# vincenthz/eccoxide

Hardware: AMD Instinct MI355X
Metric: variable-base scalarmuls/sec (batch) per GPU + achieved HBM GB/s vs roofline (higher is better)
Workload: dtype u32

## Files before the change

### eccoxide_amd/csrc/eccx_api.cpp

```cpp
#include "../../include/eccx.h"

#include <hip/hip_runtime.h>

#include <algorithm>
#include <cstring>
#include <mutex>
#include <string>
#include <thread>
#include <vector>

#include "launch.hpp"

namespace {

using eccx::CurveOps;

constexpr int NCURVES = 6;
constexpr uint32_t K_BASE_IS_GENERATOR = 1u << 0;
constexpr uint32_t K_OUT_TABLE = 1u << 1;
constexpr uint32_t K_VALIDATE = 1u << 2;
constexpr uint32_t K_OUT_ROWS = 1u << 3;
constexpr uint32_t K_NEGATE_B = 1u << 5;
constexpr uint32_t K_CT_SCAN = 1u << 6;
constexpr uint32_t K_ONLY_MARKED = 1u << 7;
// ... 153 lines not shown
size_t ed_slab_bytes(size_t n) { return 2 * align16(n * 32) + align16(n) + align16(n * 64) + n * 64; }
int ensure_ed(eccx_ctx* ctx, size_t n, EdSlab* out) {
  const int rc = grow_slab(ctx, &ctx->ed, &ctx->ed_cap, ed_slab_bytes(n));
  if (rc || !out) return rc;
  out->u1 = ctx->ed;
  out->u2 = out->u1 + align16(n * 32);
  out->lflags = out->u2 + align16(n * 32);
  out->keys = out->lflags + align16(n);
  out->pts = out->keys + align16(n * 64);
  return ECCX_OK;
}

int norm_grid(const eccx_ctx* ctx, size_t n) {
  size_t tile = (size_t)eccx::LAUNCH_WG * 8;
  size_t tiles = (n + tile - 1) / tile;
  return (int)std::max<size_t>(1, std::min(tiles, (size_t)ctx->cus * 4));
}

int flat_grid(const eccx_ctx* ctx, size_t n) {
  size_t need = (n + eccx::LAUNCH_WG - 1) / eccx::LAUNCH_WG;
  return (int)std::max<size_t>(1, std::min(need, (size_t)ctx->cus * 8));
}

int launch_var(eccx_ctx* ctx, const CurveOps* ops, size_t n, const uint8_t* d_scalars, const uint8_t* d_points,
               uint8_t* d_out, uint8_t* d_flags, uint8_t* d_proj, uint32_t kopts, bool mirror, hipStream_t s,
               bool glv = false, bool ct = false, bool ct_prime = false) {
  if (n == 0) return ECCX_OK;
  if (ct && ops->var_ct && !d_proj && d_points && !(kopts & (K_OUT_TABLE | K_BASE_IS_GENERATOR))) {
    const bool ed = ops->info.edwards != 0;
    const bool prime = ct_prime && ops->var_ct_prime;
    const int grid = prime ? ops->var_ct_prime_grid(ctx->cus, n) : ops->var_ct_grid(ctx->cus, n);
    const int grid2 = std::min(ops->var_grid ? ops->var_grid(ctx->cus, n) : grid_for(ctx, n), ctx->cus);
    int rc = ensure_scratch(ctx, ed ? ops->info.row5_words : ops->coz_row_words, grid);
    if (rc) return rc;
    if (!ed) {
      rc = ensure_scratch(ctx, ops->info.row_words, grid2);
      if (rc) return rc;
    }
    rc = ensure_rows(ctx, ops, n);
    if (rc) return rc;
    HIP_TRY(ctx, (prime ? ops->var_ct_prime : ops->var_ct)(grid, s, n, d_scalars, d_points, ctx->jac, d_flags, ctx->scratch,
                                                           kopts & ~K_CT_SCAN));
    HIP_TRY(ctx, ops->to_affine_var(norm_grid(ctx, n), s, n, ctx->jac, d_out, d_flags));
    if (!ed)
      HIP_TRY(ctx, ops->var(grid2, s, n, d_scalars, d_points, d_out, d_flags, nullptr, ctx->scratch,
                            (kopts & K_VALIDATE) | K_CT_SCAN | K_ONLY_MARKED));
    return ECCX_OK;
  }
  const bool fast = !mirror && ops->var_fast && !d_proj && !(kopts & K_OUT_TABLE);
  if (fast && ops->var_coz && d_points && !(kopts & K_BASE_IS_GENERATOR)) {
    const int g = (glv || ops->var_glv_default) ? 1 : 0;
    const int grid = ops->var_coz_grid(ctx->cus, n, g);
    const int grid2 = ops->var_fast_grid ? ops->var_fast_grid(ctx->cus, n) : grid_for(ctx, n);
    int rc = ensure_scratch(ctx, ops->coz_row_words, grid);
    if (rc) return rc;
    rc = ensure_scratch(ctx, ops->info.row5_words, grid2);
    if (rc) return rc;
    rc = ensure_rows(ctx, ops, n);
    if (rc) return rc;
    HIP_TRY(ctx, ops->var_coz(grid, s, n, d_scalars, d_points, ctx->jac, d_flags, ctx->scratch, kopts, g));
    HIP_TRY(ctx, ops->var_fast(grid2, s, n, d_scalars, d_points, ctx->jac, d_flags, ctx->scratch, kopts | K_ONLY_MARKED));
    HIP_TRY(ctx, ops->to_affine_var(norm_grid(ctx, n), s, n, ctx->jac, d_out, d_flags));
    return ECCX_OK;
  }
  int grid = fast ? (ops->var_fast_grid ? ops->var_fast_grid(ctx->cus, n) : grid_for(ctx, n))
                  : (ops->var_grid ? ops->var_grid(ctx->cus, n) : grid_for(ctx, n));
  if (fast) {
    int rc = ensure_scratch(ctx, ops->info.row5_words, grid);
    if (rc) return rc;
    rc = ensure_rows(ctx, ops, n);
    if (rc) return rc;
    HIP_TRY(ctx, ops->var_fast(grid, s, n, d_scalars, d_points, ctx->jac, d_flags, ctx->scratch, kopts));
    HIP_TRY(ctx, ops->to_affine_var(norm_grid(ctx, n), s, n, ctx->jac, d_out, d_flags));
    return ECCX_OK;
  }
  if (ops->info.row_words) {
    int rc = ensure_scratch(ctx, ops->info.row_words, grid);
    if (rc) return rc;
  }
  if (!d_proj && !(kopts & K_OUT_TABLE) && ops->to_affine_hom) {
    int rc = ensure_rows(ctx, ops, n);
    if (rc) return rc;
    HIP_TRY(ctx, ops->var(grid, s, n, d_scalars, d_points, reinterpret_cast<uint8_t*>(ctx->jac), d_flags, nullptr,
                          ctx->scratch, kopts | K_OUT_ROWS));
    HIP_TRY(ctx, ops->to_affine_hom(norm_grid(ctx, n), s, n, ctx->jac, d_out, d_flags));
    return ECCX_OK;
  }
  HIP_TRY(ctx, ops->var(grid, s, n, d_scalars, d_points, d_out, d_flags, d_proj, ctx->scratch, kopts));
  return ECCX_OK;
}

std::vector<uint8_t> comb_scalars(const CurveOps* ops) {
  int sb = ops->info.sb, nw = 2 * sb;
  std::vector<uint8_t> k((size_t)nw * 16 * sb, 0);
  for (int w = 0; w < nw; ++w)
    for (int d = 0; d < 16; ++d) {
      uint8_t* row = k.data() + ((size_t)w * 16 + d) * sb;
      row[sb - 1 - w / 2] = (uint8_t)((w & 1) ? (d << 4) : d);
    }
  return k;
}

struct DevMem {
  std::vector<void*> ptrs;
  ~DevMem() {
    for (void* p : ptrs)
      if (p) (void)hipFree(p);
// ... 229 lines not shown
    prev_done = done; prev_lo = lo; prev_cnt = cnt;
  }
  TRY2_(copy_out(prev_lo, prev_cnt, prev_done));
  TRY2_(hipStreamSynchronize(s_out));
  if (s_out != ctx->stream) TRY2_(hipStreamSynchronize(ctx->stream));
#undef TRY2_
  return ECCX_OK;
}
template <class Launch>
int host_pipeline(eccx_ctx* ctx, size_t n, const HostIn* ins, int nins, const HostOut* outs, int nouts, bool chunked,
                  Launch launch) {
  return host_pipeline_x(ctx, n, ins, nins, outs, nouts, chunked, launch, [](size_t, size_t, hipStream_t) { return hipSuccess; });
}

int run_host(eccx_ctx* ctx, int curve, bool base, size_t n, const uint8_t* scalars, const uint8_t* points,
             uint8_t* out, uint8_t* flags, uint8_t* proj, uint32_t opts) {
  const CurveOps* ops = ops_of(curve);
  if (!ctx) return ECCX_ERR_ARG;
  if (!ops) return curve_err(ctx);
  if (n == 0) return ECCX_OK;
  if (!scalars || !out || !flags || (!base && !points)) return arg_err(ctx, "null buffer");
  HIP_TRY(ctx, hipSetDevice(ctx->device));
  size_t sb = ops->info.sb, pb = 2 * (size_t)ops->info.fb;
  uint8_t *d_k = nullptr, *d_p = nullptr, *d_o = nullptr, *d_f = nullptr, *d_j = nullptr;
  int rc = ensure_io(ctx, IO_K, n * sb, &d_k);
  if (!rc) rc = ensure_io(ctx, IO_O, n * pb, &d_o);
  if (!rc) rc = ensure_io(ctx, IO_F, n, &d_f);
  if (!rc && !base) rc = ensure_io(ctx, IO_P, n * pb, &d_p);
  if (!rc && proj) rc = ensure_io(ctx, IO_J, n * proj_bytes(ops), &d_j);
  if (rc) return rc;
  const bool chunked = !proj && (!base || ((opts & ECCX_CT_SCAN) && !(opts & (ECCX_MIRROR_REFERENCE | ECCX_TABLE_IN_L2))));
  const HostIn ins[2] = {{d_k, scalars, sb}, {d_p, base ? nullptr : points, pb}};
  const HostOut outs[3] = {{out, d_o, pb}, {flags, d_f, 1}, {proj, d_j, proj_bytes(ops)}};
  return host_pipeline(ctx, n, ins, 2, outs, 3, chunked, [&](size_t lo, size_t cnt) {
    if (base) return eccx_scalarmul_base_dev(ctx, curve, cnt, d_k + lo * sb, d_o + lo * pb, d_f + lo, d_j, opts, ctx->stream);
    return eccx_scalarmul_var_dev(ctx, curve, cnt, d_k + lo * sb, d_p + lo * pb, d_o + lo * pb, d_f + lo, d_j, opts, ctx->stream);
  });
}

int verify_shape(eccx_ctx* ctx, int curve, const CurveOps* ops, size_t n, const uint8_t* d_u1, const uint8_t* d_u2,
                 const uint8_t* d_q, uint8_t* d_out, uint8_t* d_flags, uint32_t opts, hipStream_t s) {
  HIP_TRY(ctx, hipSetDevice(ctx->device));
  int rc = ensure_comb(ctx, curve, ops, s);
  if (rc) return rc;
  if (!ctx->comb_u[curve]) return ECCX_ERR_HIP;
  const int grid = ops->var_fast_grid ? ops->var_fast_grid(ctx->cus, n) : grid_for(ctx, n);
  rc = ensure_scratch(ctx, ops->info.row5_words, grid);
  if (rc) return rc;
  rc = ensure_rows(ctx, ops, n);
  if (rc) return rc;
  const uint32_t kopts = kopts_of(opts) | ((opts & ECCX_SUBTRACT) ? K_NEGATE_B : 0u);
  if (ops->var_coz_fused) {
    const int gridc = ops->var_coz_fused_grid(ctx->cus, n);
    rc = ensure_scratch(ctx, ops->coz_row_words, gridc);
    if (rc) return rc;
    HIP_TRY(ctx, ops->var_coz_fused(gridc, s, n, d_u2, d_q, ctx->jac, d_flags, ctx->scratch, kopts, d_u1, ctx->comb_u[curve]));
  }
  HIP_TRY(ctx, ops->var_fused(grid, s, n, d_u2, d_q, ctx->jac, d_flags, ctx->scratch,
                              kopts | (ops->var_coz_fused ? K_ONLY_MARKED : 0u), d_u1, ctx->comb_u[curve]));
  HIP_TRY(ctx, ((opts & ECCX_OUT_X_ONLY) ? ops->to_affine_x : ops->to_affine_var)(norm_grid(ctx, n), s, n, ctx->jac, d_out,
                                                                                  d_flags));
  return ECCX_OK;
}

int ecdsa_args(eccx_ctx* ctx, const CurveOps* ops, size_t digest_bytes, uint32_t opts) {
  if (!ops->ecdsa_prepare || !ops->ecdsa_finish)
    return arg_err(ctx, "eccx_ecdsa_verify: ECDSA is defined on p256r1, p384r1, p521r1 and p256k1");
  if (opts & ~(uint32_t)ECCX_PUBKEY_SEC1) return arg_err(ctx, "eccx_ecdsa_verify: ECCX_PUBKEY_SEC1 is the only option");
  if (digest_bytes > 2 * (size_t)ops->info.sb) return arg_err(ctx, "eccx_ecdsa_verify: digest_bytes must be 0 .. 2*SB");
  return ECCX_OK;
}

int run_sharded(eccx_ctx** ctxs, int nctx, int curve, bool base, size_t n, const uint8_t* scalars,
                const uint8_t* points, uint8_t* out, uint8_t* flags, uint32_t opts) {
  const CurveOps* ops = ops_of(curve);
  if (!ops) return ECCX_ERR_CURVE;
  if (!ctxs || nctx < 1) return ECCX_ERR_ARG;
  for (int i = 0; i < nctx; ++i)
    if (!ctxs[i]) return ECCX_ERR_ARG;
  size_t sb = ops->info.sb, pb = 2 * (size_t)ops->info.fb;
  std::vector<int> rcs((size_t)nctx, ECCX_OK);
  std::vector<std::thread> th;
  for (int g = 0; g < nctx; ++g) {
    size_t lo = n * (size_t)g / (size_t)nctx, hi = n * (size_t)(g + 1) / (size_t)nctx;
    th.emplace_back([=, &rcs]() {
      rcs[(size_t)g] = run_host(ctxs[g], curve, base, hi - lo, scalars + lo * sb, base ? nullptr : points + lo * pb,
                                out + lo * pb, flags + lo, nullptr, opts);
    });
  }
  for (auto& t : th) t.join();
  for (int rc : rcs)
    if (rc) return rc;
  return ECCX_OK;
}

}

extern "C" {

int eccx_field_bytes(int curve) {
  const CurveOps* o = ops_of(curve);
  return o ? o->info.fb : ECCX_ERR_CURVE;
}
int eccx_scalar_bytes(int curve) {
  const CurveOps* o = ops_of(curve);
  return o ? o->info.sb : ECCX_ERR_CURVE;
}
// ... 59 lines not shown
  if (!ctx) return "null context";
  static thread_local std::string copy;
  eccx_ctx* c = const_cast<eccx_ctx*>(ctx);
  std::lock_guard<std::mutex> g(c->err_mu);
  copy = c->err;
  return copy.c_str();
}

const char* eccx_strerror(int code) {
  switch (code) {
    case ECCX_OK: return "ok";
    case ECCX_ERR_CURVE: return "unknown curve id";
    case ECCX_ERR_ARG: return "bad argument";
    case ECCX_ERR_HIP: return "HIP runtime error";
    case ECCX_ERR_NOMEM: return "out of device memory";
    default: return "unknown error";
  }
}

int eccx_prepare(eccx_ctx* ctx, int curve, uint32_t what) {
  const CurveOps* ops = ops_of(curve);
  if (!ctx) return ECCX_ERR_ARG;
  if (!ops) return curve_err(ctx);
  HIP_TRY(ctx, hipSetDevice(ctx->device));
  int rc = ECCX_OK;
  if (what & ECCX_PREP_BASE) rc = ensure_comb(ctx, curve, ops, ctx->stream);
  if (!rc && (what & ECCX_PREP_BASE_LDS)) {
    if (!ops->base_lds || !ops->lds_convert) {
      ctx->set_err("ECCX_PREP_BASE_LDS: this curve has no LDS-resident fixed-base kernel (edwards25519 only)");
      return ECCX_ERR_ARG;
    }
    rc = ensure_comb_lds(ctx, curve, ops, ctx->stream);
  }
  if (!rc && (what & ECCX_PREP_CT)) rc = ensure_comb_ct(ctx, curve, ops, ctx->stream, false);
  if (!rc && (what & ECCX_PREP_CT_GATHER)) rc = ensure_comb_ct(ctx, curve, ops, ctx->stream, true);
  return rc;
}

int eccx_reserve(eccx_ctx* ctx, int curve, size_t max_n, uint32_t what) {
  const CurveOps* ops = ops_of(curve);
  if (!ctx) return ECCX_ERR_ARG;
  if (!ops) return curve_err(ctx);
  if (max_n == 0) return ECCX_OK;
  HIP_TRY(ctx, hipSetDevice(ctx->device));
  int rc = ensure_rows(ctx, ops, max_n);
  if (rc) return rc;
  if (what & (ECCX_PREP_VAR | ECCX_PREP_ECDSA | ECCX_PREP_ED25519)) {
    const int grid = ops->var_fast_grid ? ops->var_fast_grid(ctx->cus, max_n) : grid_for(ctx, max_n);
    rc = ensure_scratch(ctx, ops->info.row5_words, grid);
    if (rc) return rc;
    if (ops->var_coz) {
      int g = std::max(ops->var_coz_grid(ctx->cus, max_n, 0), ops->var_coz_grid(ctx->cus, max_n, 1));
      if (ops->var_coz_fused_grid) g = std::max(g, ops->var_coz_fused_grid(ctx->cus, max_n));
      rc = ensure_scratch(ctx, ops->coz_row_words, g);
      if (rc) return rc;
    }
  }
  if (what & ECCX_PREP_HOST) {
    const size_t pb = 2 * (size_t)ops->info.fb, sbytes = (size_t)ops->info.sb;
    uint8_t* dummy = nullptr;
    rc = ensure_io(ctx, IO_K, max_n * std::max(pb, sbytes), &dummy);
    if (!rc) rc = ensure_io(ctx, IO_P, max_n * pb, &dummy);
    if (!rc) rc = ensure_io(ctx, IO_O, max_n * pb, &dummy);
    if (!rc) rc = ensure_io(ctx, IO_F, max_n, &dummy);
    if (!rc) rc = ensure_io(ctx, IO_J, max_n * sbytes, &dummy);
    if (!rc) rc = ensure_io(ctx, IO_A, max_n, &dummy);
    if (!rc) rc = ensure_io(ctx, IO_B, max_n, &dummy);
    if (rc) return rc;
  }
  if ((what & ECCX_PREP_CT) && ops->var_ct) {
    const bool ed = ops->info.edwards != 0;
    rc = ensure_scratch(ctx, ed ? ops->info.row5_words : ops->coz_row_words, ops->var_ct_grid(ctx->cus, max_n));
    if (rc) return rc;
    if (ops->var_ct_prime) {
      rc = ensure_scratch(ctx, ops->coz_row_words, ops->var_ct_prime_grid(ctx->cus, max_n));
      if (rc) return rc;
    }
    if (!ed) {
      const int grid2 = std::min(ops->var_grid ? ops->var_grid(ctx->cus, max_n) : grid_for(ctx, max_n), ctx->cus);
      rc = ensure_scratch(ctx, ops->info.row_words, grid2);
      if (rc) return rc;
    }
  }
  if ((what & ECCX_PREP_ECDSA) && ops->ecdsa_prepare) {
    rc = ensure_ecdsa(ctx, ops, max_n, nullptr);
    if (rc) return rc;
  }
  if ((what & ECCX_PREP_ED25519) && ops->ed_verify_prepare) {
    rc = ensure_ed(ctx, max_n, nullptr);
    if (rc) return rc;
  }
  const bool mirror_slab = (what & ECCX_PREP_MIRROR) || ((what & ECCX_PREP_CT) && !ops->var_ct);
  if (mirror_slab && ops->info.row_words) {
    const int grid = ops->var_grid ? ops->var_grid(ctx->cus, max_n) : grid_for(ctx, max_n);
    rc = ensure_scratch(ctx, ops->info.row_words, grid);
    if (rc) return rc;
  }
  return ECCX_OK;
}

size_t eccx_device_bytes(const eccx_ctx* ctx) {
  if (!ctx) return 0;
  eccx_ctx* c = const_cast<eccx_ctx*>(ctx);
  std::lock_guard<std::mutex> g1(c->comb_mu);
  std::lock_guard<std::mutex> g2(c->scratch_mu);
  size_t io = 0;
  for (size_t b : c->io_cap) io += b;
// ... 486 lines not shown
```

### eccoxide_amd/csrc/k_weierstrass.inc

```
#include "kernels_codec.hpp"
#include "kernels_coz.hpp"
#include "launch.hpp"
#ifdef ECCX_ORDER
#include "kernels_ecdsa.hpp"
#endif
#ifndef ECCX_CODEC_FORMAT
#define ECCX_CODEC_FORMAT FORMAT_SEC1
#endif

namespace eccx {
namespace {
hipError_t var_(int grid, hipStream_t s, size_t n, const uint8_t* scalars, const uint8_t* points, uint8_t* out,
                uint8_t* flags, uint8_t* proj, uint32_t* scratch, uint32_t opts) {
  hipLaunchKernelGGL(k_scalarmul_var_mirror_unsat<ECCX_CURVE_U>, dim3(grid), dim3(WG), 0, s, n, scalars, points, out, flags, proj, scratch,
                     opts);
  return hipGetLastError();
}
hipError_t base_(int grid, hipStream_t s, size_t n, const uint8_t* scalars, const uint32_t* table, uint8_t* out,
                 uint8_t* flags, uint8_t* proj, uint32_t opts) {
  hipLaunchKernelGGL(k_scalarmul_base<ECCX_CURVE>, dim3(grid), dim3(WG), 0, s, n, scalars, table, out, flags, proj, opts);
  return hipGetLastError();
}
hipError_t var_fast_(int grid, hipStream_t s, size_t n, const uint8_t* scalars, const uint8_t* points, uint32_t* jac,
                     uint8_t* flags, uint32_t* scratch, uint32_t opts) {
// ... 136 lines not shown
                        const uint8_t* b_inf, uint32_t* rows, uint8_t* flags, uint32_t opts) {
  hipLaunchKernelGGL(k_point_add_unsat<ECCX_CURVE_U>, dim3(grid), dim3(WG), 0, s, n, a, a_inf, b, b_inf, rows, flags, opts);
  return hipGetLastError();
}
hipError_t to_affine_add_u_(int grid, hipStream_t s, size_t n, const uint32_t* rows, uint8_t* out, uint8_t* flags) {
  hipLaunchKernelGGL((k_batch_to_affine_unsat<ECCX_CURVE_U, NORM_HOMOGENEOUS, to_affine_add_u(ECCX_CURVE::L)>), dim3(grid), dim3(WG), 0, s,
                     n, rows, out, flags);
  return hipGetLastError();
}
template <int F>
hipError_t decompress_raw_(int grid, hipStream_t s, size_t n, const uint8_t* enc, uint8_t* out, uint8_t* flags) {
  if constexpr (F == FORMAT_ZCASH) {
    hipLaunchKernelGGL(k_point_from_uncompressed<ECCX_CURVE_U>, dim3(grid), dim3(WG), 0, s, n, enc, out, flags);
    return hipGetLastError();
  } else {
    return hipErrorNotSupported;
  }
}
template <int F>
hipError_t compress_raw_(int grid, hipStream_t s, size_t n, const uint8_t* xy, const uint8_t* inf, uint8_t* out) {
  if constexpr (F == FORMAT_ZCASH) {
    hipLaunchKernelGGL((k_point_compress<ECCX_CURVE, FORMAT_ZCASH_RAW>), dim3(grid), dim3(WG), 0, s, n, xy, inf, out);
    return hipGetLastError();
  } else {
    return hipErrorNotSupported;
  }
}
#ifdef ECCX_ORDER
static_assert(ECCX_ORDER::SB == ECCX_CURVE::SB && ECCX_CURVE::FB == ECCX_CURVE::SB, "x-coordinates and scalars share a width");
hipError_t ecdsa_prepare_(int grid, hipStream_t s, size_t n, const uint8_t* digests, int digest_bytes, const uint8_t* sigs,
                          const uint8_t* key_flags, uint8_t* u1, uint8_t* u2, uint8_t* verdicts) {
  hipLaunchKernelGGL(k_ecdsa_prepare<ECCX_ORDER>, dim3(grid), dim3(WG), 0, s, n, digests, digest_bytes, sigs, key_flags, u1, u2,
                     verdicts);
  return hipGetLastError();
}
hipError_t ecdsa_finish_(int grid, hipStream_t s, size_t n, const uint8_t* sigs, const uint8_t* xs, const uint8_t* lflags,
                         uint8_t* verdicts) {
  hipLaunchKernelGGL(k_ecdsa_finish<ECCX_ORDER>, dim3(grid), dim3(WG), 0, s, n, sigs, xs, lflags, verdicts);
  return hipGetLastError();
}
#endif
}
const CurveOps& ECCX_OPS_NAME() {
  static const CurveOps o = [] {
    CurveOps t = {{ECCX_CURVE::FB, ECCX_CURVE::SB, ECCX_CURVE::L, 2 * ECCX_CURVE::L, urow3_words<ECCX_CURVE_U>(), 0, urow_words<ECCX_CURVE_U>(),
                              (urow3_words<ECCX_CURVE_U>() > row_words<ECCX_CURVE::L>() ? urow3_words<ECCX_CURVE_U>() : row_words<ECCX_CURVE::L>())}, var_, base_, var_fast_, nullptr, to_affine_hom_, var_grid_, var_fast_grid_, to_affine_var_, point_add_, utable_words<ECCX_CURVE_U>(), comb_bits<ECCX_CURVE_U>(), comb_convert_, base_unsat_, 0, 0, 0, 0, nullptr, var_fused_,
                              enc_bytes<ECCX_CURVE, ECCX_CODEC_FORMAT>(), decompress_, compress_,
                              ECCX_CODEC_FORMAT == FORMAT_ZCASH ? decompress_raw_<ECCX_CODEC_FORMAT> : nullptr,
                              ECCX_CODEC_FORMAT == FORMAT_ZCASH ? compress_raw_<ECCX_CODEC_FORMAT> : nullptr,
                              point_add_u_, to_affine_add_u_};
    t.var_coz = var_coz_t<COZ_HAS_GLV>;
    t.var_coz_grid = var_coz_grid_t<COZ_HAS_GLV>;
    t.coz_row_words = urowc_words<ECCX_CURVE_U>();
    t.var_coz_fused = var_coz_fused_;
    t.var_coz_fused_grid = var_coz_fused_grid_;
    t.ct_bits = ct_base_bits<ECCX_CURVE_U>();
    t.ct_windows = ct_base_windows<ECCX_CURVE_U>();
    t.ct_entries = ct_base_entries<ECCX_CURVE_U>();
    t.ct_entry_words = ct_entry_words<ECCX_CURVE_U>();
    t.ct_convert = ct_convert_;
    t.base_ct = base_ct_;
    t.ctg_bits = ct_base_bits<ECCX_CURVE_U, true>();
    t.ctg_windows = ct_base_windows<ECCX_CURVE_U, true>();
    t.ctg_entries = ct_base_entries<ECCX_CURVE_U, true>();
    t.base_ctg = base_ctg_;
    t.var_ct = var_ct_;
    t.var_ct_prime = ECCX_CURVE::PRIME_ORDER ? nullptr : var_ct_prime_;
    t.var_ct_prime_grid = var_ct_prime_grid_;
    t.var_ct_grid = var_ct_grid_;
    t.to_affine_x = to_affine_x_;
#ifdef ECCX_ORDER
    t.ecdsa_prepare = ecdsa_prepare_;
    t.ecdsa_finish = ecdsa_finish_;
#endif
#ifdef ECCX_EXTRA_OPS
    ECCX_EXTRA_OPS(t);
#endif
    return t;
  }();
  return o;
}
}
```

### eccoxide_amd/csrc/kernels_coz.hpp

```cpp
#pragma once
#include <type_traits>
#include "inv_gcd.hpp"
#include "kernels_ct.hpp"

namespace eccx {

struct NoGlv {
  static constexpr int K_BITS = 0;
};
struct PrimeOrderBases : NoGlv {};

template <class G>
ECCX_DEV void glv_split(uint32_t (&k1)[5], uint32_t (&k2)[5], const uint8_t* __restrict__ kb) {
  uint32_t k[8];
#pragma unroll
  for (int i = 0; i < 8; ++i) {
    const uint8_t* b = kb + 28 - 4 * i;
    k[i] = ((uint32_t)b[0] << 24) | ((uint32_t)b[1] << 16) | ((uint32_t)b[2] << 8) | (uint32_t)b[3];
  }
  uint32_t prod[13];
#pragma unroll
  for (int i = 0; i < 13; ++i) prod[i] = 0;
#pragma unroll
  for (int i = 0; i < 8; ++i) {
// ... 290 lines not shown
template <class CU>
ECCX_DEV void ujac_dbl_affine(U<CU, 1, 3>& x3, U<CU, 1, 3>& y3, U<CU, 1, 3>& z3, U<CU, 1, 3>& sv, U<CU, 1, 3>& y8v,
                              const U<CU, 1, 3>& px, const U<CU, 1, 3>& py) {
  const auto xx = u_sqr(px);
  const auto yy = u_sqr(py);
  const auto yyyy = u_sqr(yy);
  const auto xyy = u_mul(px, yy);
  const auto s2 = u_add(xyy, xyy);
  sv = u_reduce(u_add(s2, s2));
  const auto y4 = u_add(yyyy, yyyy);
  const auto y8 = u_add(y4, y4);
  y8v = u_reduce(u_add(y8, y8));
  if constexpr (CU::Sat::A0 == 1) {
    const auto m = u_reduce(u_add(u_add(xx, xx), xx));
    x3 = u_reduce(u_sub(u_sub(u_sqr(m), sv), sv));
    y3 = u_reduce(u_sub(u_mul(m, u_sub(sv, x3)), y8v));
  } else {
    U<CU, 1, 3> one;
#pragma unroll
    for (int i = 0; i < CU::N; ++i) one.v[i] = CU::ONE[i];
    const auto xm = u_sub(xx, one);
    const auto m = u_reduce(u_add(u_add(xm, xm), xm));
    x3 = u_reduce(u_sub(u_sub(u_sqr(m), sv), sv));
    y3 = u_reduce(u_sub(u_mul(m, u_sub(sv, x3)), y8v));
  }
  z3 = u_reduce(u_add(py, py));
}

template <class CU, int WB, bool ASSUME_PRIME = false>
constexpr int coz_full_windows() {
  using CS = typename CU::Sat;
  constexpr int NWIN = (8 * CS::SB + 1 + WB - 1) / WB;
  return (CS::PRIME_ORDER || ASSUME_PRIME) ? (8 * CS::SB - CS::NBITS + 1) / WB + 1 : NWIN;
}
#ifndef ECCX_CT_VAR_BITS
#define ECCX_CT_VAR_BITS 4
#endif

#ifndef ECCX_COZ_OCC_U14
#define ECCX_COZ_OCC_U14 3
#endif
#ifndef ECCX_COZ_OCC_BLS
#define ECCX_COZ_OCC_BLS 2
#endif
#ifndef ECCX_COZ_OCC_U9
#define ECCX_COZ_OCC_U9 4
#endif
template <class CU, bool GLV>
constexpr int coz_occupancy() {
  return CU::N <= 9 ? ECCX_COZ_OCC_U9
                    : (CU::N <= 14 ? (GLV ? ECCX_OCC_U14 : (CU::KIND == UK_MONT ? ECCX_COZ_OCC_BLS : ECCX_COZ_OCC_U14)) : ECCX_OCC_U18);
}

template <class CU, class G, bool GLV, bool FUSED = false, int WB = 5, bool CT = false>
__global__ void __launch_bounds__(WG, (coz_occupancy<CU, GLV>())) k_scalarmul_coz_unsat(size_t n, const uint8_t* __restrict__ scalars,
                                                                                 const uint8_t* __restrict__ points,
                                                                                 uint32_t* __restrict__ rows_out,
                                                                                 uint8_t* __restrict__ flags,
                                                                                 uint32_t* __restrict__ scratch, uint32_t opts,
                                                                                 const uint8_t* __restrict__ base_scalars = nullptr,
                                                                                 const uint32_t* __restrict__ utable = nullptr) {
  static_assert(!(GLV && FUSED), "the verify shape takes any curve point");
  static_assert(!(CT && FUSED), "the verify shape has no secret-scalar form");
  constexpr bool ASSUME_PRIME = std::is_same<G, PrimeOrderBases>::value;
  constexpr bool LATTICE = GlvLattice<G>::value;
  static_assert(!(LATTICE && CT), "the secret-scalar endomorphism ladder is written for the unsigned split");
  static_assert(!ASSUME_PRIME || CT, "PrimeOrderBases only narrows the secret-scalar form's collision windows");
  static_assert(WB >= 3 && WB <= 5, "table rows 1 .. 2^(WB-1) must fit the slab");
  constexpr int TBL = 1 << (WB - 1);
  using CS = typename CU::Sat;
  constexpr bool ISO = CS::A0 == 1;
  constexpr int L = CS::L;
  constexpr int N = CU::N;
  constexpr int FB = CS::FB;
  constexpr int SB = CS::SB;
  static_assert(!GLV || SB == 32, "the split is written for 256-bit scalars");
  constexpr int NWIN = GLV ? (G::K_BITS + 1 + WB - 1) / WB : (8 * SB + 1 + WB - 1) / WB;
  constexpr int WR = urowc_words<CU>();
  static_assert(!ISO || WR >= 16 + N, "row 0 holds the split scalar and zeta");
  using T = U<CU, 1, 3>;
  uint32_t* slab = scratch + ((size_t)blockIdx.x * FAST_TABLE_ROWS * WG + threadIdx.x) * (size_t)WR;
  auto row = [&](uint32_t e) { return slab + (size_t)e * WG * WR; };
  constexpr int WC = urow2_words<CU>();
  static_assert(!CT || (size_t)TBL * WC <= (size_t)(FAST_TABLE_ROWS - 1 - TBL) * WR, "the compact table must fit the free rows");
  uint32_t* cslab = scratch + ((size_t)blockIdx.x * FAST_TABLE_ROWS + (TBL + 1)) * WG * (size_t)WR + (size_t)threadIdx.x * WC;
  auto crow = [&](uint32_t e) { return cslab + (size_t)(e - 1) * WG * WC; };
  for (size_t base = (size_t)blockIdx.x * WG; base < n; base += (size_t)gridDim.x * WG) {
    const size_t gid = base + threadIdx.x;
    const bool active = gid < n;
    const size_t idx = active ? gid : n - 1;
    const uint8_t* __restrict__ k = scalars + idx * (size_t)SB;
    if constexpr (GLV) {
      uint32_t k1[5], k2[5], s1 = 0, s2 = 0;
      if constexpr (LATTICE) glv_split_lattice<G>(k1, k2, s1, s2, k);
      else glv_split<G>(k1, k2, k);
      uint4* d = reinterpret_cast<uint4*>(row(0));
      d[0] = make_uint4(k1[0], k1[1], k1[2], k1[3]);
      d[1] = make_uint4(k1[4], s1, 0u, 0u);
      d[2] = make_uint4(k2[0], k2[1], k2[2], k2[3]);
      d[3] = make_uint4(k2[4], s2, 0u, 0u);
    }
    const uint32_t* kw = row(0);

    T one;
#pragma unroll
    for (int i = 0; i < N; ++i) one.v[i] = CU::ONE[i];
    UJac<CU> q;
    bool rejected = false;
    {
      Fe<L> rx, ry;
      fe_load_be<CS>(rx, points + idx * (size_t)(2 * FB));
      fe_load_be<CS>(ry, points + idx * (size_t)(2 * FB) + FB);
      if (opts & OPT_VALIDATE) {
        Fe<L> mx, my;
        fe_to_mont<CS>(mx, rx);
        fe_to_mont<CS>(my, ry);
        rejected = !(fe_is_canonical<CS>(rx) && fe_is_canonical<CS>(ry) && on_curve<CS>(mx, my));
      }
      q.x = u_as<1, 3>(u_to_mont<CU>(rx));
      q.y = u_as<1, 3>(u_to_mont<CU>(ry));
    }
    if constexpr (FUSED) {
      if (opts & OPT_NEGATE_B) q.y = u_reduce(u_neg(q.y));
    }
    q.z = u_as<UJac<CU>::ZK, UJac<CU>::ZV>(one);
    u3_store<CU>(row(1), q.x, q.y, one);

    auto booth = [&](int w, bool second, uint32_t& d, bool& neg) {
      uint32_t w6;
      if constexpr (GLV) {
        const uint32_t* h = kw + (second ? 8 : 0);
        const int pos = WB * w - 1 + 32;
        const int wi = pos >> 5, sh = pos & 31;
        const uint32_t lo = (wi >= 1 && wi <= 5) ? h[wi - 1] : 0u;
        const uint32_t hi = (wi <= 4) ? h[wi] : 0u;
        w6 = (uint32_t)((((uint64_t)hi << 32) | lo) >> sh) & ((1u << (WB + 1)) - 1u);
        const uint32_t s = ~((w6 >> WB) - 1u);
        const uint32_t m = (((1u << (WB + 1)) - w6 - 1u) & s) | (w6 & ~s);
        d = (m >> 1) + (m & 1u);
        neg = (s & 1u) != 0;
        if constexpr (LATTICE) neg = neg != (h[5] != 0u);
      } else {
        booth_digit<WB, SB>(k, w, d, neg);
      }
    };

    bool degenerate = false;
    {
      T px = q.x, py = q.y;
      T tx, ty, ratio;
      T zacc = one;
      {
        T x3, y3, sv, y8v;
        ujac_dbl_affine<CU>(x3, y3, ratio, sv, y8v, px, py);
        degenerate = u_is_zero_mod_p(ratio);
        tx = x3;
        ty = y3;
        px = sv;
        py = y8v;
        if constexpr (!ISO) zacc = ratio;
        u3_store<CU>(row(2), tx, ty, ratio);
      }
      for (int d = 3; d <= TBL; ++d) {
        bool dz;
        uzaddu<CU>(px, py, tx, ty, ratio, dz);
        degenerate = degenerate || dz;
        if constexpr (!ISO) zacc = u_fit<1, 3>(u_mul(zacc, ratio));
        u3_store<CU>(row(d), tx, ty, ratio);
      }
      T lam = one, next = ratio;
      if constexpr (ISO) {
        if constexpr (CT) u2_store<CU, (ECCX_CT_VAR_PK != 0)>(crow(TBL), tx, ty);
        else if constexpr (GLV) u3_store<CU>(row(TBL), tx, ty, u_fit<1, 3>(u_mul_k<CU>(tx, CU::BETA)));
      } else {
        Fe<L> c;
        u_to_canonical<CU>(c, zacc);
        fe_inv_gcd<CS>(c, c);
        lam = u_as<1, 3>(u_to_mont<CU>(c));
        const T l2 = u_fit<1, 3>(u_sqr(lam));
        const T l3 = u_fit<1, 3>(u_mul(l2, lam));
        const T xt = u_fit<1, 3>(u_mul(tx, l2)), yt = u_fit<1, 3>(u_mul(ty, l3));
        if constexpr (CT) u2_store<CU, (ECCX_CT_VAR_PK != 0)>(crow(TBL), xt, yt);
        else u3_store<CU>(row(TBL), xt, yt, one);
      }
      for (int d = TBL - 1; d >= 1; --d) {
        lam = u_fit<1, 3>(u_mul(lam, next));
        T x, y;
        u3_load<CU>(x, y, next, row(d));
        const T l2 = u_fit<1, 3>(u_sqr(lam));
        const T l3 = u_fit<1, 3>(u_mul(l2, lam));
        const T xs = u_fit<1, 3>(u_mul(x, l2));
        const T ys = u_fit<1, 3>(u_mul(y, l3));
        if constexpr (CT) u2_store<CU, (ECCX_CT_VAR_PK != 0)>(crow(d), xs, ys);
        else if constexpr (GLV) u3_store<CU>(row(d), xs, ys, u_fit<1, 3>(u_mul_k<CU>(xs, CU::BETA)));
        else u3_store<CU>(row(d), xs, ys, one);
      }
      if constexpr (ISO) {
        uint32_t* zdst = row(0) + 16;
#pragma unroll
        for (int i = 0; i < N; ++i) zdst[i] = lam.v[i];
      }
    }

    if constexpr (CT) {
      constexpr int FULLW = GLV ? 1 : coz_full_windows<CU, WB, ASSUME_PRIME>();
      constexpr int HALVES = GLV ? 2 : 1;
      auto lookup = [&](int w, bool second, T& ex, T& ey, uint32_t& d) {
        bool neg;
        booth(w, second, d, neg);
        neg = neg != second;
#if ECCX_CT_VAR_PK
        {
          uint64_t acc[N];
#pragma unroll
          for (int p = 0; p < N; ++p) acc[p] = 0;
#pragma unroll 2
          for (int j = 1; j <= TBL; ++j) {
            uint32_t m;
            asm("v_cndmask_b32_e64 %0, 0, 1.0, %1" : "=v"(m) : "s"(__builtin_amdgcn_uicmp(d, (uint32_t)j, 32 )));
            const uint64_t m2 = m;
            const uint4* src = reinterpret_cast<const uint4*>(crow(j));
            uint4 v[WC / 4];
#pragma unroll
            for (int c = 0; c < WC / 4; ++c) v[c] = src[c];
#pragma unroll
            for (int p = 0; p < N; ++p) {
              const uint4 qv = v[p / 2];
              ct_fsel2(acc[p], (p & 1) ? (((uint64_t)qv.w << 32) | qv.z) : (((uint64_t)qv.y << 32) | qv.x), m2);
            }
          }
#pragma unroll
// ... 130 lines not shown
          bool neg;
          booth(win, second, d, neg);
          if (second && !LATTICE) neg = !neg;
          T ex, ey;
          if constexpr (GLV) {
            T eb;
            u3_load<CU>(ex, ey, eb, row(d ? d : 1));
            if (second) ex = eb;
          } else {
            u2_load<CU>(ex, ey, row(d ? d : 1));
          }
          const bool q_inf = u_limbs_all_zero(q.z);
          const bool e_skip = (d == 0);
          UJac<CU> sum;
          bool hz, rz;
          ujac_madd_signed<CU>(sum, hz, rz, q, ex, ey, neg);
          const bool same_x = hz && !q_inf && !e_skip;
          fix_lane = same_x && rz;
          if (same_x && !rz) u_set_zero(sum.z);
          if (__builtin_amdgcn_ballot_w64(q_inf) != 0) {
            U<CU, 2, 4> sy;
            u_select(sy, neg, u_neg(ey), u_as<2, 4>(ey));
            u_select(sum.x, q_inf, ex, sum.x);
            u_select(sum.y, q_inf, u_reduce(sy), sum.y);
            u_select(sum.z, q_inf, u_as<UJac<CU>::ZK, UJac<CU>::ZV>(one), sum.z);
          }
          const bool keep = e_skip || fix_lane;
          u_select(q.x, keep, q.x, sum.x);
          u_select(q.y, keep, q.y, sum.y);
          u_select(q.z, keep, q.z, sum.z);
          fix_pending = __builtin_amdgcn_ballot_w64(fix_lane) != 0;
          step_done = !fix_pending;
        }
        if (step_done) {
          if (sub < LAST_SUB) {
            ++sub;
          } else {
            sub = 0;
            --win;
          }
        }
      }
    }
    if constexpr (ISO) {
      T zeta;
      const uint32_t* zsrc = row(0) + 16;
#pragma unroll
      for (int i = 0; i < N; ++i) zeta.v[i] = zsrc[i];
      q.z = u_fit<UJac<CU>::ZK, UJac<CU>::ZV>(u_mul(q.z, zeta));
    }
    if constexpr (FUSED) ucomb_accumulate<CU, false>(q, base_scalars + idx * (size_t)SB, utable);
    if (active) {
      u3_store<CU>(rows_out + idx * (size_t)urow3_words<CU>(), q.x, q.y, u_fit<1, 3>(q.z));
      flags[idx] = rejected ? 2 : (degenerate ? FLAG_REDO : 0);
    }
  }
}

}
```

### eccoxide_amd/csrc/launch.hpp

```cpp
#pragma once
#ifndef ECCX_NORM_U8
#define ECCX_NORM_U8 16
#endif
#ifndef ECCX_NORM_UBIG
#define ECCX_NORM_UBIG 8
#endif
#include <hip/hip_runtime.h>
#include <stddef.h>
#include <stdint.h>

namespace eccx {

struct CurveInfo {
  int fb;
  int sb;
  int limbs;
  int table_words;
  int row_words;
  int edwards;
  int row5_words;
  int jac_words;
};

struct CurveOps {
  CurveInfo info;
  hipError_t (*var)(int grid, hipStream_t s, size_t n, const uint8_t* scalars, const uint8_t* points, uint8_t* out,
                    uint8_t* flags, uint8_t* proj, uint32_t* scratch, uint32_t opts);
  hipError_t (*base)(int grid, hipStream_t s, size_t n, const uint8_t* scalars, const uint32_t* table, uint8_t* out,
                     uint8_t* flags, uint8_t* proj, uint32_t opts);
  hipError_t (*var_fast)(int grid, hipStream_t s, size_t n, const uint8_t* scalars, const uint8_t* points,
                         uint32_t* jac, uint8_t* flags, uint32_t* scratch, uint32_t opts);
  hipError_t (*base_lds)(int cus, hipStream_t s, size_t n, const uint8_t* scalars, const uint32_t* table,
                         uint32_t* rows, uint8_t* flags);
  hipError_t (*to_affine_hom)(int grid, hipStream_t s, size_t n, const uint32_t* rows, uint8_t* out, uint8_t* flags);
  int (*var_grid)(int cus, size_t n);
  int (*var_fast_grid)(int cus, size_t n);
  hipError_t (*to_affine_var)(int grid, hipStream_t s, size_t n, const uint32_t* rows, uint8_t* out, uint8_t* flags);
  hipError_t (*point_add)(int grid, hipStream_t s, size_t n, const uint8_t* a, const uint8_t* a_inf, const uint8_t* b,
                          const uint8_t* b_inf, uint32_t* rows, uint8_t* flags, uint32_t opts);
  int utable_words;
  int comb_bits;
  hipError_t (*comb_convert)(hipStream_t s, size_t entries, const uint8_t* affine, uint32_t* utable);
  hipError_t (*base_unsat)(int grid, hipStream_t s, size_t n, const uint8_t* scalars, const uint32_t* utable,
                           uint32_t* rows, uint8_t* flags);
  int lds_bits, lds_windows, lds_digits, lds_entry_words;
  hipError_t (*lds_convert)(hipStream_t s, size_t entries, const uint8_t* affine, uint32_t* table);
  hipError_t (*var_fused)(int grid, hipStream_t s, size_t n, const uint8_t* u2, const uint8_t* q, uint32_t* rows,
                          uint8_t* flags, uint32_t* scratch, uint32_t opts, const uint8_t* u1, const uint32_t* utable);
  int enc_bytes;
  hipError_t (*decompress)(int grid, hipStream_t s, size_t n, const uint8_t* enc, uint8_t* out, uint8_t* flags);
  hipError_t (*compress)(int grid, hipStream_t s, size_t n, const uint8_t* xy, const uint8_t* inf, uint8_t* out);
  hipError_t (*decompress_raw)(int grid, hipStream_t s, size_t n, const uint8_t* enc, uint8_t* out, uint8_t* flags);
  hipError_t (*compress_raw)(int grid, hipStream_t s, size_t n, const uint8_t* xy, const uint8_t* inf, uint8_t* out);
  hipError_t (*point_add_u)(int grid, hipStream_t s, size_t n, const uint8_t* a, const uint8_t* a_inf, const uint8_t* b,
                            const uint8_t* b_inf, uint32_t* rows, uint8_t* flags, uint32_t opts);
  hipError_t (*to_affine_add_u)(int grid, hipStream_t s, size_t n, const uint32_t* rows, uint8_t* out, uint8_t* flags);
  hipError_t (*var_coz)(int grid, hipStream_t s, size_t n, const uint8_t* scalars, const uint8_t* points, uint32_t* rows,
                        uint8_t* flags, uint32_t* scratch, uint32_t opts, int glv);
  int (*var_coz_grid)(int cus, size_t n, int glv);
  int coz_row_words;
  hipError_t (*var_coz_fused)(int grid, hipStream_t s, size_t n, const uint8_t* u2, const uint8_t* q, uint32_t* rows, uint8_t* flags,
                              uint32_t* scratch, uint32_t opts, const uint8_t* u1, const uint32_t* utable);
  int (*var_coz_fused_grid)(int cus, size_t n);
  hipError_t (*subgroup_check)(int grid, hipStream_t s, size_t n, uint8_t* xy, uint8_t* flags);
  int ct_bits, ct_windows, ct_entries, ct_entry_words;
  int ctg_bits, ctg_windows, ctg_entries;
  hipError_t (*ct_convert)(hipStream_t s, size_t entries, const uint8_t* affine, uint32_t* table);
  hipError_t (*base_ct)(int grid, hipStream_t s, size_t n, const uint8_t* scalars, const uint32_t* table, uint32_t* rows,
                        uint8_t* flags);
  hipError_t (*base_ctg)(int grid, hipStream_t s, size_t n, const uint8_t* scalars, const uint32_t* table, uint32_t* rows,
                         uint8_t* flags);
  hipError_t (*var_ct)(int grid, hipStream_t s, size_t n, const uint8_t* scalars, const uint8_t* points, uint32_t* rows,
                       uint8_t* flags, uint32_t* scratch, uint32_t opts);
  int (*var_ct_grid)(int cus, size_t n);
  hipError_t (*var_ct_prime)(int grid, hipStream_t s, size_t n, const uint8_t* scalars, const uint8_t* points, uint32_t* rows,
                             uint8_t* flags, uint32_t* scratch, uint32_t opts);
  int (*var_ct_prime_grid)(int cus, size_t n);
  hipError_t (*to_affine_x)(int grid, hipStream_t s, size_t n, const uint32_t* rows, uint8_t* out, uint8_t* flags);
  int var_glv_default;
  hipError_t (*ecdsa_prepare)(int grid, hipStream_t s, size_t n, const uint8_t* digests, int digest_bytes, const uint8_t* sigs,
                              const uint8_t* key_flags, uint8_t* u1, uint8_t* u2, uint8_t* verdicts);
  hipError_t (*ecdsa_finish)(int grid, hipStream_t s, size_t n, const uint8_t* sigs, const uint8_t* xs, const uint8_t* lflags,
                             uint8_t* verdicts);
  hipError_t (*ed_verify_prepare)(int grid, hipStream_t s, size_t n, const uint8_t* msgs, const uint64_t* offsets,
                                  const uint8_t* sigs, const uint8_t* pubkeys, const uint8_t* key_flags, uint8_t* u1, uint8_t* u2,
                                  uint8_t* verdicts);
  hipError_t (*ed_verify_finish)(int grid, hipStream_t s, size_t n, const uint8_t* sigs, const uint8_t* pts, uint8_t* verdicts);
};
constexpr int to_affine_u(int limbs) { return limbs <= 8 ? ECCX_NORM_U8 : ECCX_NORM_UBIG; }
#ifndef ECCX_NORM_ADD_U8
#define ECCX_NORM_ADD_U8 ECCX_NORM_U8
#endif
#ifndef ECCX_NORM_ADD_UBIG
#define ECCX_NORM_ADD_UBIG ECCX_NORM_UBIG
#endif
constexpr int to_affine_add_u(int limbs) { return limbs <= 8 ? ECCX_NORM_ADD_U8 : ECCX_NORM_ADD_UBIG; }

const CurveOps& ops_P256();
const CurveOps& ops_P384();
const CurveOps& ops_P521();
const CurveOps& ops_BLS12_381();
const CurveOps& ops_ED25519();
const CurveOps& ops_P256K1();

hipError_t launch_x25519_ladder(int grid, hipStream_t s, size_t n, const uint8_t* scalars, const uint8_t* u,
                                uint32_t* rows, uint8_t* flags, uint32_t opts);
hipError_t launch_x25519_to_u(int grid, hipStream_t s, size_t n, const uint32_t* rows, uint8_t* out, uint8_t* flags);

constexpr int LAUNCH_WG = 256;

template <class K>
inline int occupancy_per_cu(K kernel) {
  int per_cu = 0;
  if (hipOccupancyMaxActiveBlocksPerMultiprocessor(&per_cu, kernel, LAUNCH_WG, 0) != hipSuccess || per_cu < 1) per_cu = 1;
  return per_cu;
}
inline int persistent_grid(int per_cu, int cus, size_t n) {
  size_t need = (n + LAUNCH_WG - 1) / LAUNCH_WG;
  size_t cap = (size_t)cus * (size_t)per_cu;
  size_t g = need < cap ? need : cap;
  return (int)(g ? g : 1);
}

}
```

Before: 74.65 million.

## Batch the coZ table inversion across several grid-stride iterations with Montgomery's trick

Result: no change. 74.94 million (median of 4 runs) (+0.4%).

```diff
diff --git a/eccoxide_amd/csrc/eccx_api.cpp b/eccoxide_amd/csrc/eccx_api.cpp
--- a/eccoxide_amd/csrc/eccx_api.cpp
+++ b/eccoxide_amd/csrc/eccx_api.cpp
@@ -229,7 +229,7 @@
     const int g = (glv || ops->var_glv_default) ? 1 : 0;
     const int grid = ops->var_coz_grid(ctx->cus, n, g);
     const int grid2 = ops->var_fast_grid ? ops->var_fast_grid(ctx->cus, n) : grid_for(ctx, n);
-    int rc = ensure_scratch(ctx, ops->coz_row_words, grid);
+    int rc = ensure_scratch(ctx, eccx::coz_slab_row_words(*ops), grid);
     if (rc) return rc;
     rc = ensure_scratch(ctx, ops->info.row5_words, grid2);
     if (rc) return rc;
@@ -565,7 +565,7 @@
   const uint32_t kopts = kopts_of(opts) | ((opts & ECCX_SUBTRACT) ? K_NEGATE_B : 0u);
   if (ops->var_coz_fused) {
     const int gridc = ops->var_coz_fused_grid(ctx->cus, n);
-    rc = ensure_scratch(ctx, ops->coz_row_words, gridc);
+    rc = ensure_scratch(ctx, eccx::coz_slab_row_words(*ops), gridc);
     if (rc) return rc;
     HIP_TRY(ctx, ops->var_coz_fused(gridc, s, n, d_u2, d_q, ctx->jac, d_flags, ctx->scratch, kopts, d_u1, ctx->comb_u[curve]));
   }
@@ -731,7 +731,7 @@
     if (ops->var_coz) {
       int g = std::max(ops->var_coz_grid(ctx->cus, max_n, 0), ops->var_coz_grid(ctx->cus, max_n, 1));
       if (ops->var_coz_fused_grid) g = std::max(g, ops->var_coz_fused_grid(ctx->cus, max_n));
-      rc = ensure_scratch(ctx, ops->coz_row_words, g);
+      rc = ensure_scratch(ctx, eccx::coz_slab_row_words(*ops), g);
       if (rc) return rc;
     }
   }
diff --git a/eccoxide_amd/csrc/k_weierstrass.inc b/eccoxide_amd/csrc/k_weierstrass.inc
--- a/eccoxide_amd/csrc/k_weierstrass.inc
+++ b/eccoxide_amd/csrc/k_weierstrass.inc
@@ -212,6 +212,7 @@
     t.var_coz = var_coz_t<COZ_HAS_GLV>;
     t.var_coz_grid = var_coz_grid_t<COZ_HAS_GLV>;
     t.coz_row_words = urowc_words<ECCX_CURVE_U>();
+    t.coz_units = coz_inv_units<ECCX_CURVE_U, false>();
     t.var_coz_fused = var_coz_fused_;
     t.var_coz_fused_grid = var_coz_fused_grid_;
     t.ct_bits = ct_base_bits<ECCX_CURVE_U>();
diff --git a/eccoxide_amd/csrc/kernels_coz.hpp b/eccoxide_amd/csrc/kernels_coz.hpp
--- a/eccoxide_amd/csrc/kernels_coz.hpp
+++ b/eccoxide_amd/csrc/kernels_coz.hpp
@@ -366,6 +366,21 @@
                     : (CU::N <= 14 ? (GLV ? ECCX_OCC_U14 : (CU::KIND == UK_MONT ? ECCX_COZ_OCC_BLS : ECCX_COZ_OCC_U14)) : ECCX_OCC_U18);
 }
 
+#ifndef ECCX_COZ_INV_UNITS_U9
+#define ECCX_COZ_INV_UNITS_U9 1
+#endif
+#ifndef ECCX_COZ_INV_UNITS_U14
+#define ECCX_COZ_INV_UNITS_U14 1
+#endif
+#ifndef ECCX_COZ_INV_UNITS_U18
+#define ECCX_COZ_INV_UNITS_U18 4
+#endif
+template <class CU, bool CT>
+constexpr int coz_inv_units() {
+  return (CU::Sat::A0 == 1 || CT) ? 1
+                                  : (CU::N <= 9 ? ECCX_COZ_INV_UNITS_U9 : (CU::N <= 14 ? ECCX_COZ_INV_UNITS_U14 : ECCX_COZ_INV_UNITS_U18));
+}
+
 template <class CU, class G, bool GLV, bool FUSED = false, int WB = 5, bool CT = false>
 __global__ void __launch_bounds__(WG, (coz_occupancy<CU, GLV>())) k_scalarmul_coz_unsat(size_t n, const uint8_t* __restrict__ scalars,
                                                                                  const uint8_t* __restrict__ points,
@@ -393,13 +408,98 @@
   constexpr int WR = urowc_words<CU>();
   static_assert(!ISO || WR >= 16 + N, "row 0 holds the split scalar and zeta");
   using T = U<CU, 1, 3>;
-  uint32_t* slab = scratch + ((size_t)blockIdx.x * FAST_TABLE_ROWS * WG + threadIdx.x) * (size_t)WR;
-  auto row = [&](uint32_t e) { return slab + (size_t)e * WG * WR; };
+  constexpr int GI = coz_inv_units<CU, CT>();
+  static_assert(GI == 1 || (!ISO && !GLV && 2 * N <= WR), "row 0 of a slot holds zeta and the group's prefix product");
+  uint32_t* slab = scratch + ((size_t)blockIdx.x * GI * FAST_TABLE_ROWS * WG + threadIdx.x) * (size_t)WR;
+  auto srow = [&](int s, uint32_t e) { return slab + ((size_t)s * FAST_TABLE_ROWS + e) * WG * WR; };
   constexpr int WC = urow2_words<CU>();
   static_assert(!CT || (size_t)TBL * WC <= (size_t)(FAST_TABLE_ROWS - 1 - TBL) * WR, "the compact table must fit the free rows");
   uint32_t* cslab = scratch + ((size_t)blockIdx.x * FAST_TABLE_ROWS + (TBL + 1)) * WG * (size_t)WR + (size_t)threadIdx.x * WC;
   auto crow = [&](uint32_t e) { return cslab + (size_t)(e - 1) * WG * WC; };
+  int s = 0;
   for (size_t base = (size_t)blockIdx.x * WG; base < n; base += (size_t)gridDim.x * WG) {
+    auto build = [&](int slot, size_t idx, UJac<CU>& q, bool& rejected, bool& degenerate, T& tx, T& ty, T& ratio, T& zacc) {
+      auto row = [&](uint32_t e) { return srow(slot, e); };
+      T one;
+#pragma unroll
+      for (int i = 0; i < N; ++i) one.v[i] = CU::ONE[i];
+      {
+        Fe<L> rx, ry;
+        fe_load_be<CS>(rx, points + idx * (size_t)(2 * FB));
+        fe_load_be<CS>(ry, points + idx * (size_t)(2 * FB) + FB);
+        if (opts & OPT_VALIDATE) {
+          Fe<L> mx, my;
+          fe_to_mont<CS>(mx, rx);
+          fe_to_mont<CS>(my, ry);
+          rejected = !(fe_is_canonical<CS>(rx) && fe_is_canonical<CS>(ry) && on_curve<CS>(mx, my));
+        }
+        q.x = u_as<1, 3>(u_to_mont<CU>(rx));
+        q.y = u_as<1, 3>(u_to_mont<CU>(ry));
+      }
+      if constexpr (FUSED) {
+        if (opts & OPT_NEGATE_B) q.y = u_reduce(u_neg(q.y));
+      }
+      q.z = u_as<UJac<CU>::ZK, UJac<CU>::ZV>(one);
+      u3_store<CU>(row(1), q.x, q.y, one);
+
+      T px = q.x, py = q.y;
+      zacc = one;
+      {
+        T x3, y3, sv, y8v;
+        ujac_dbl_affine<CU>(x3, y3, ratio, sv, y8v, px, py);
+        degenerate = u_is_zero_mod_p(ratio);
+        tx = x3;
+        ty = y3;
+        px = sv;
+        py = y8v;
+        if constexpr (!ISO) zacc = ratio;
+        u3_store<CU>(row(2), tx, ty, ratio);
+      }
+      for (int d = 3; d <= TBL; ++d) {
+        bool dz;
+        uzaddu<CU>(px, py, tx, ty, ratio, dz);
+        degenerate = degenerate || dz;
+        if constexpr (!ISO) zacc = u_fit<1, 3>(u_mul(zacc, ratio));
+        u3_store<CU>(row(d), tx, ty, ratio);
+      }
+    };
+
+    if (GI > 1 && s == 0) {
+      T one;
+#pragma unroll
+      for (int i = 0; i < N; ++i) one.v[i] = CU::ONE[i];
+      const size_t stride = (size_t)gridDim.x * WG;
+      T zpre = one;
+      int ns = 0;
+#pragma unroll 1
+      for (; ns < GI && base + ns * stride < n; ++ns) {
+        const size_t gid = base + ns * stride + threadIdx.x;
+        const bool active = gid < n;
+        const size_t idx = active ? gid : n - 1;
+        UJac<CU> q;
+        bool rejected = false, degenerate = false;
+        T tx, ty, ratio, zacc, z;
+        build(ns, idx, q, rejected, degenerate, tx, ty, ratio, zacc);
+        u_select(z, active && !degenerate, zacc, one);
+        u3_store<CU>(srow(ns, 0), z, zpre, one);
+        zpre = u_fit<1, 3>(u_mul(zpre, z));
+        if (active) flags[idx] = rejected ? 2 : (degenerate ? FLAG_REDO : 0);
+      }
+      Fe<L> c;
+      u_to_canonical<CU>(c, zpre);
+      fe_inv_gcd<CS>(c, c);
+      T inv = u_as<1, 3>(u_to_mont<CU>(c));
+#pragma unroll 1
+      for (int j = ns - 1; j >= 0; --j) {
+        T z, pre, unused;
+        u3_load<CU>(z, pre, unused, srow(j, 0));
+        const T lz = u_fit<1, 3>(u_mul(inv, pre));
+        inv = u_fit<1, 3>(u_mul(inv, z));
+        u3_store<CU>(srow(j, 0), lz, pre, z);
+      }
+    }
+
+    auto row = [&](uint32_t e) { return srow(s, e); };
     const size_t gid = base + threadIdx.x;
     const bool active = gid < n;
     const size_t idx = active ? gid : n - 1;
@@ -421,24 +521,10 @@
     for (int i = 0; i < N; ++i) one.v[i] = CU::ONE[i];
     UJac<CU> q;
     bool rejected = false;
-    {
-      Fe<L> rx, ry;
-      fe_load_be<CS>(rx, points + idx * (size_t)(2 * FB));
-      fe_load_be<CS>(ry, points + idx * (size_t)(2 * FB) + FB);
-      if (opts & OPT_VALIDATE) {
-        Fe<L> mx, my;
-        fe_to_mont<CS>(mx, rx);
-        fe_to_mont<CS>(my, ry);
-        rejected = !(fe_is_canonical<CS>(rx) && fe_is_canonical<CS>(ry) && on_curve<CS>(mx, my));
-      }
-      q.x = u_as<1, 3>(u_to_mont<CU>(rx));
-      q.y = u_as<1, 3>(u_to_mont<CU>(ry));
-    }
-    if constexpr (FUSED) {
-      if (opts & OPT_NEGATE_B) q.y = u_reduce(u_neg(q.y));
-    }
-    q.z = u_as<UJac<CU>::ZK, UJac<CU>::ZV>(one);
-    u3_store<CU>(row(1), q.x, q.y, one);
+    bool degenerate = false;
+    T tx, ty, ratio, zacc;
+    if constexpr (GI == 1) build(s, idx, q, rejected, degenerate, tx, ty, ratio, zacc);
+    else u3_load<CU>(tx, ty, ratio, row(TBL));
 
     auto booth = [&](int w, bool second, uint32_t& d, bool& neg) {
       uint32_t w6;
@@ -459,38 +545,21 @@
       }
     };
 
-    bool degenerate = false;
     {
-      T px = q.x, py = q.y;
-      T tx, ty, ratio;
-      T zacc = one;
-      {
-        T x3, y3, sv, y8v;
-        ujac_dbl_affine<CU>(x3, y3, ratio, sv, y8v, px, py);
-        degenerate = u_is_zero_mod_p(ratio);
-        tx = x3;
-        ty = y3;
-        px = sv;
-        py = y8v;
-        if constexpr (!ISO) zacc = ratio;
-        u3_store<CU>(row(2), tx, ty, ratio);
-      }
-      for (int d = 3; d <= TBL; ++d) {
-        bool dz;
-        uzaddu<CU>(px, py, tx, ty, ratio, dz);
-        degenerate = degenerate || dz;
-        if constexpr (!ISO) zacc = u_fit<1, 3>(u_mul(zacc, ratio));
-        u3_store<CU>(row(d), tx, ty, ratio);
-      }
       T lam = one, next = ratio;
       if constexpr (ISO) {
         if constexpr (CT) u2_store<CU, (ECCX_CT_VAR_PK != 0)>(crow(TBL), tx, ty);
         else if constexpr (GLV) u3_store<CU>(row(TBL), tx, ty, u_fit<1, 3>(u_mul_k<CU>(tx, CU::BETA)));
       } else {
-        Fe<L> c;
-        u_to_canonical<CU>(c, zacc);
-        fe_inv_gcd<CS>(c, c);
-        lam = u_as<1, 3>(u_to_mont<CU>(c));
+        if constexpr (GI == 1) {
+          Fe<L> c;
+          u_to_canonical<CU>(c, zacc);
+          fe_inv_gcd<CS>(c, c);
+          lam = u_as<1, 3>(u_to_mont<CU>(c));
+        } else {
+          T pre, z;
+          u3_load<CU>(lam, pre, z, row(0));
+        }
         const T l2 = u_fit<1, 3>(u_sqr(lam));
         const T l3 = u_fit<1, 3>(u_mul(l2, lam));
         const T xt = u_fit<1, 3>(u_mul(tx, l2)), yt = u_fit<1, 3>(u_mul(ty, l3));
@@ -727,9 +796,10 @@
     if constexpr (FUSED) ucomb_accumulate<CU, false>(q, base_scalars + idx * (size_t)SB, utable);
     if (active) {
       u3_store<CU>(rows_out + idx * (size_t)urow3_words<CU>(), q.x, q.y, u_fit<1, 3>(q.z));
-      flags[idx] = rejected ? 2 : (degenerate ? FLAG_REDO : 0);
-    }
-  }
-}
-
-}
+      if constexpr (GI == 1) flags[idx] = rejected ? 2 : (degenerate ? FLAG_REDO : 0);
+    }
+    if constexpr (GI > 1) s = s + 1 == GI ? 0 : s + 1;
+  }
+}
+
+}
diff --git a/eccoxide_amd/csrc/launch.hpp b/eccoxide_amd/csrc/launch.hpp
--- a/eccoxide_amd/csrc/launch.hpp
+++ b/eccoxide_amd/csrc/launch.hpp
@@ -59,6 +59,7 @@
                         uint8_t* flags, uint32_t* scratch, uint32_t opts, int glv);
   int (*var_coz_grid)(int cus, size_t n, int glv);
   int coz_row_words;
+  int coz_units;
   hipError_t (*var_coz_fused)(int grid, hipStream_t s, size_t n, const uint8_t* u2, const uint8_t* q, uint32_t* rows, uint8_t* flags,
                               uint32_t* scratch, uint32_t opts, const uint8_t* u1, const uint32_t* utable);
   int (*var_coz_fused_grid)(int cus, size_t n);
@@ -115,6 +116,7 @@
   if (hipOccupancyMaxActiveBlocksPerMultiprocessor(&per_cu, kernel, LAUNCH_WG, 0) != hipSuccess || per_cu < 1) per_cu = 1;
   return per_cu;
 }
+inline int coz_slab_row_words(const CurveOps& o) { return o.coz_row_words * o.coz_units; }
 inline int persistent_grid(int per_cu, int cus, size_t n) {
   size_t need = (n + LAUNCH_WG - 1) / LAUNCH_WG;
   size_t cap = (size_t)cus * (size_t)per_cu;
```
